# NikolausDemmel/rootba

Hardware: NVIDIA H100
Metric: ms/LM-iter (linearize+QR+PCG) on BAL at 1/2/4/8 H100 vs CPU ref (lower is better)
Workload: dtype f32

## Files before the change

### rootba_b200/csrc/assembled.cuh

```cuda
#pragma once

#include "kernels.cuh"

namespace rba {

template <class S>
__global__ void __launch_bounds__(256) k_rcs_terms(const S* __restrict__ panel, const AsmTerm* __restrict__ terms, long long nt,
                                                   int damping, S* __restrict__ stage, const int* __restrict__ done) {
  using V2 = typename ST<S>::V2;
  if (*done) return;
  const int lane = threadIdx.x & 31;
  const int g = lane / 9, p = lane - 9 * g;
  if (lane >= 27) return;
  const long long warps = (long long)gridDim.x * (blockDim.x >> 5);
  for (long long w = 3 * (blockIdx.x * (long long)(blockDim.x >> 5) + (threadIdx.x >> 5)) + g; w < nt; w += 3 * warps) {
    const AsmTerm at = terms[w];
    const int n = at.meta & 0x7fff, lg = (at.meta >> 15) & 7, KP = at.meta >> 18, G = 1 << lg;
    const int ia = at.ij & 0xffff, ib = at.ij >> 16;
    const int ca = 9 * ia + p, pa = ca >> 1;
    const int off_a = 2 * ((pa >> lg) * 32 + (pa & (G - 1))) + (ca & 1);
    const int cb0 = 9 * ib, pb0 = cb0 >> 1;
    const bool odd = cb0 & 1;
    int off_b[5];
#pragma unroll
    for (int k = 0; k < 5; ++k) off_b[k] = ((pb0 + k) >> lg) * 32 + ((pb0 + k) & (G - 1));
    const size_t rstride = (size_t)KP * 64;
    const S* __restrict__ lmp = panel + at.base;
    const int r0 = damping ? 2 * n - 3 : 0, r1 = damping ? 2 * n : 2 * n - 3;
    S acc[9];
#pragma unroll
    for (int q = 0; q < 9; ++q) acc[q] = 0;
#pragma unroll 3
    for (int r = r0; r < r1; ++r) {
      const S* row = lmp + (size_t)r * rstride;
      const V2* row2 = reinterpret_cast<const V2*>(row);
      const S va = __ldg(row + off_a);
      V2 b[5];
#pragma unroll
      for (int k = 0; k < 5; ++k) b[k] = __ldg(row2 + off_b[k]);
      const S el[10] = {b[0].x, b[0].y, b[1].x, b[1].y, b[2].x, b[2].y, b[3].x, b[3].y, b[4].x, b[4].y};
#pragma unroll
      for (int q = 0; q < 9; ++q) acc[q] = fma(va, odd ? el[q + 1] : el[q], acc[q]);
    }
    S* o = stage + 81 * (size_t)w + 9 * p;
#pragma unroll
    for (int q = 0; q < 9; ++q) o[q] = acc[q];
  }
}

template <class S>
__global__ void k_rcs_combine(const int* __restrict__ blk_ptr, const int* __restrict__ wpos, int nblk, const S* __restrict__ stage,
                              S* __restrict__ out, const int* __restrict__ done) {
  if (*done) return;
  const long long i = blockIdx.x * (long long)blockDim.x + threadIdx.x;
  if (i >= 81LL * nblk) return;
  const int bi = (int)(i / 81), e = (int)(i - 81LL * bi);
  const S* st = stage + e;
  S s = 0;
  for (int t = blk_ptr[bi]; t < blk_ptr[bi + 1]; ++t) s += st[81 * (size_t)wpos[t]];
  out[i] = s;
}

constexpr int DMP_WARPS = 4;
constexpr int DMP_BATCH = 16;
template <class S>
__global__ void __launch_bounds__(DMP_WARPS * 32) k_rcs_damping(const int* __restrict__ blk_ptr, const int2* __restrict__ terms, int nblk,
                                                                 const S* __restrict__ dmp, const S* __restrict__ base,
                                                                 const int2* __restrict__ pos, S* __restrict__ out,
                                                                 const int* __restrict__ done) {
  constexpr int B = DMP_BATCH, NV = 28 * sizeof(S) / 16;
  constexpr int ROUNDS = (2 * B * NV + 31) / 32;
  __shared__ __align__(16) S rec[DMP_WARPS][B][2][28];
  if (*done) return;
  const int w = threadIdx.x >> 5, lane = threadIdx.x & 31;
  const int bi = blockIdx.x * DMP_WARPS + w;
  if (bi >= nblk) return;
  const bool own = lane < 27;
  const int p = lane / 3, q = 3 * (lane - 3 * p);
  S s[3] = {0, 0, 0};
  if (own) {
#pragma unroll
    for (int u = 0; u < 3; ++u) s[u] = base[81 * (size_t)bi + 3 * lane + u];
  }
  int4* rv = reinterpret_cast<int4*>(&rec[w][0][0][0]);
  const int t1 = blk_ptr[bi + 1];
  for (int t0 = blk_ptr[bi]; t0 < t1; t0 += B) {
    const int nb = min(B, t1 - t0);
    int4 v[ROUNDS];
#pragma unroll
    for (int c = 0; c < ROUNDS; ++c) {
      const int i = lane + 32 * c, r = i / NV, k = i - r * NV;
      v[c] = make_int4(0, 0, 0, 0);
      if (i < 2 * nb * NV) {
        const int2 tt = __ldg(terms + t0 + (r >> 1));
        v[c] = __ldg(reinterpret_cast<const int4*>(dmp + 28 * (size_t)(r & 1 ? tt.y : tt.x)) + k);
      }
    }
#pragma unroll
    for (int c = 0; c < ROUNDS; ++c)
      if (lane + 32 * c < 2 * nb * NV) rv[lane + 32 * c] = v[c];
    __syncwarp();
    if (own) {
      for (int j = 0; j < nb; ++j) {
        const S* a = rec[w][j][0];
        const S* b = rec[w][j][1];
#pragma unroll
        for (int u = 0; u < 3; ++u) {
          S t = fma(a[p], b[q + u], S(0));
          t = fma(a[9 + p], b[9 + q + u], t);
          t = fma(a[18 + p], b[18 + q + u], t);
          s[u] += t;
        }
      }
    }
    __syncwarp();
  }
  if (own) {
    S* o = out + 81 * (size_t)pos[bi].x + 3 * lane;
#pragma unroll
    for (int u = 0; u < 3; ++u) o[u] = s[u];
  }
}

template <class S>
__global__ void k_rcs_mirror(const int2* __restrict__ pos, int nblk, S* val, const int* __restrict__ done) {
  if (*done) return;
  const long long i = blockIdx.x * (long long)blockDim.x + threadIdx.x;
  if (i >= 81LL * nblk) return;
  const int bi = (int)(i / 81), e = (int)(i - 81LL * bi);
  const int2 ps = pos[bi];
  if (ps.y >= 0) val[81 * (size_t)ps.y + e] = val[81 * (size_t)ps.x + 9 * (e % 9) + e / 9];
}

constexpr int SPMV_NS = 3;
template <class S>
__global__ void __launch_bounds__(SPMV_CLASSES * 32) k_rcs_spmv(const SpmvChunk* __restrict__ chunks, const int* __restrict__ chunk_ptr,
                                                                 const int* __restrict__ col, const S* __restrict__ val,
                                                                 const S* __restrict__ x, S* __restrict__ y, const int* done, int pdl) {
  constexpr int CH = SPMV_STAGE_BYTES / (81 * (int)sizeof(S)), U = CH / SPMV_CLASSES;
  constexpr int VB = CH * 81 * (int)sizeof(S) + 16;
  constexpr int XWIN = sizeof(S) == 4 ? 256 : 128;
  static_assert(CH % SPMV_CLASSES == 0 && VB % 16 == 0 && XWIN >= CH, "k_rcs_spmv stage layout");
// ... 127 lines not shown
```

### rootba_b200/csrc/layout.hpp

```cpp
#pragma once

#include <algorithm>
#include <cmath>
#include <cstdint>
#include <limits>
#include <numeric>
#include <string>
#include <utility>
#include <vector>

namespace rba {

struct TileInfo {
  long long panel_off;
  int slot_base;
  int lm_base;
  short n;
  short G;
  short KP;
  short nvalid;
};

struct MatvecItem {
  int tile;
// ... 237 lines not shown
    if (!L.csr_y_is_obs) build_csr(nc, L.nyslots, ycam, L.csr_y);
    L.pb_cam_item_ptr.assign(nc + 1, 0);
    for (int c = 0; c < nc; ++c) {
      L.pb_cam_item_ptr[c] = (int)L.pb_items.size();
      for (int b = L.csr_obs.cam_ptr[c]; b < L.csr_obs.cam_ptr[c + 1]; b += PB_SEG_LEN)
        L.pb_items.push_back({c, b, std::min(b + PB_SEG_LEN, L.csr_obs.cam_ptr[c + 1])});
    }
    L.pb_cam_item_ptr[nc] = (int)L.pb_items.size();
  }
  for (const TileInfo& T : L.tiles) {
    const int W = 32 / T.G;
    const int CS = (2 * T.G * T.KP) | 1;
    L.k4_scratch_per_warp = std::max(L.k4_scratch_per_warp, T.KP > kp_max ? 2 * 64 * (int)T.KP : W * CS);
  }
  return "";
}

struct IntPair {
  int x, y;
};

struct PairList {
  std::vector<int> slot0, nn;
  std::vector<IntPair> blk_cam;
  std::vector<int> blk_ptr;
  std::vector<IntPair> terms;
  std::vector<int> wpos;
};

inline std::string build_pair_list(const Layout& L, PairList& P) {
  const int nl = L.nl_local, nc = L.nc;
  P = PairList();
  P.slot0.resize(nl); P.nn.resize(nl);
  long long nt = 0;
  for (int lm = 0; lm < nl; ++lm) {
    const int sidx = L.sorted_of_lm[lm];
    const TileInfo& T = L.tiles[L.tile_of_sorted[sidx]];
    P.slot0[lm] = T.slot_base + (sidx - T.lm_base) * T.n;
    P.nn[lm] = T.n;
    nt += (long long)T.n * (T.n + 1) / 2;
  }
  if (nt > std::numeric_limits<int>::max()) return "more than 2^31 camera-pair terms";
  std::vector<IntPair> raw;
  raw.reserve((size_t)nt);
  for (int lm = 0; lm < nl; ++lm)
    for (int a = 0; a < P.nn[lm]; ++a)
      for (int b = 0; b <= a; ++b) raw.push_back({P.slot0[lm] + a, P.slot0[lm] + b});
  std::vector<int> idx(raw.size()), tmp(raw.size());
  std::iota(idx.begin(), idx.end(), 0);
  std::vector<long long> cnt((size_t)nc + 1);
  auto pass = [&](const std::vector<int>& src, std::vector<int>& dst, bool by_a) {
    std::fill(cnt.begin(), cnt.end(), 0LL);
    for (int w : src) ++cnt[L.slot_cam[by_a ? raw[w].x : raw[w].y] + 1];
    for (int c = 0; c < nc; ++c) cnt[c + 1] += cnt[c];
    for (int w : src) dst[cnt[L.slot_cam[by_a ? raw[w].x : raw[w].y]]++] = w;
  };
  pass(idx, tmp, false);
  pass(tmp, idx, true);
  tmp.clear(); tmp.shrink_to_fit();
  P.terms.resize(raw.size());
  for (size_t t = 0; t < idx.size(); ++t) P.terms[t] = raw[idx[t]];
  P.wpos.swap(idx);
  for (size_t t = 0; t < P.terms.size(); ++t) {
    const IntPair cc{L.slot_cam[P.terms[t].x], L.slot_cam[P.terms[t].y]};
    if (t == 0 || cc.x != P.blk_cam.back().x || cc.y != P.blk_cam.back().y) {
      P.blk_cam.push_back(cc);
      P.blk_ptr.push_back((int)t);
    }
  }
  P.blk_ptr.push_back((int)P.terms.size());
  return "";
}

struct AsmTerm {
  long long base;
  int ij, meta;
};
inline AsmTerm pack_asm_term(long long base, int ia, int ib, int n, int G, int KP) {
  int lg = 0;
  while ((1 << lg) < G) ++lg;
  return {base, ia | ib << 16, n | lg << 15 | KP << 18};
}

constexpr long long ASM_STAGE_BYTES = (long long)2 << 30;

inline int asm_switch_iteration(long long nt, long long panel_scalars, long long s_bytes, int scalar_size) {
  const double staged = 4.0 * (double)nt * 81 * scalar_size, saved = (double)panel_scalars * scalar_size - (double)s_bytes;
  return 1 + (int)std::ceil(2.0 * staged / std::max(saved, 1.0));
}

constexpr int SPMV_CLASSES = 4;
constexpr int SPMV_STAGE_BYTES = 32 * 81 * 4;
constexpr int spmv_chunk_blocks(int scalar_size) { return SPMV_STAGE_BYTES / (81 * scalar_size); }
struct SpmvChunk {
  int row, kb, ke;
  int flags;
};
constexpr int SPMV_FIRST = 1, SPMV_LAST = 2;
struct SpmvDeal {
  int ctas = 0;
  std::vector<int> chunk_ptr;
  std::vector<SpmvChunk> chunks;
};
inline void deal_spmv(const std::vector<int>& row_ptr, int ctas, int chunk_blocks, SpmvDeal& D) {
  D = SpmvDeal();
  const int nrows = (int)row_ptr.size() - 1;
  D.ctas = std::max(1, std::min(ctas, nrows));
  std::vector<long long> cost((size_t)std::max(nrows, 0));
  for (int r = 0; r < nrows; ++r) cost[r] = row_ptr[r + 1] - row_ptr[r];
  const std::vector<int> order = deal_lpt(cost, D.ctas);
  D.chunk_ptr.assign((size_t)D.ctas + 1, 0);
  for (int b = 0; b < D.ctas; ++b) {
    D.chunk_ptr[b] = (int)D.chunks.size();
    for (size_t k = b; k < order.size(); k += D.ctas) {
      const int r = order[k];
      if (r < 0) break;
      const int k0 = row_ptr[r], k1 = row_ptr[r + 1];
      int kb = k0;
      do {
        const int ke = std::min(k1, kb + chunk_blocks);
        D.chunks.push_back({r, kb, ke, (kb == k0 ? SPMV_FIRST : 0) | (ke == k1 ? SPMV_LAST : 0)});
        kb = ke;
      } while (kb < k1);
    }
  }
  D.chunk_ptr[D.ctas] = (int)D.chunks.size();
}

struct AsmPlan {
  long long nt = 0, nblk = 0, nnzb = 0, s_bytes = 0, device_bytes = 0;
  bool fits = false;
  int switch_iteration = 0;
  std::vector<int> row_ptr;
  std::vector<int> col;
  std::vector<IntPair> pos;
  std::vector<AsmTerm> terms;
  SpmvDeal spmv;
};

inline void plan_assembled(const Layout& L, const PairList& P, int scalar_size, AsmPlan& A, int spmv_ctas = 0) {
  A = AsmPlan();
  const int nc = L.nc;
  A.nblk = (long long)P.blk_cam.size();
  A.nt = (long long)P.terms.size();
  long long ndiag = 0;
  for (const IntPair& c : P.blk_cam) ndiag += c.x == c.y;
  A.nnzb = 2 * A.nblk - ndiag;
  A.s_bytes = A.nnzb * 81 * scalar_size;
  A.switch_iteration = asm_switch_iteration(A.nt, L.panel_scalars, A.s_bytes, scalar_size);
  A.fits = 4 * A.s_bytes <= L.panel_scalars * scalar_size && 81 * A.nt * scalar_size <= ASM_STAGE_BYTES;
  if (!A.fits) return;
  A.device_bytes = A.s_bytes + 16 + (A.nblk + A.nt) * 81 * scalar_size + A.nt * (long long)(sizeof(AsmTerm) + sizeof(int) + sizeof(IntPair)) +
                   (A.nblk + 1 + A.nnzb) * (long long)sizeof(int) + A.nblk * (long long)sizeof(IntPair);
  A.row_ptr.assign((size_t)nc + 1, 0);
  A.col.resize((size_t)A.nnzb);
  for (const IntPair& c : P.blk_cam) { ++A.row_ptr[c.x + 1]; if (c.x != c.y) ++A.row_ptr[c.y + 1]; }
  for (int c = 0; c < nc; ++c) A.row_ptr[c + 1] += A.row_ptr[c];
  std::vector<int> fill(A.row_ptr.begin(), A.row_ptr.end() - 1);
  A.pos.resize((size_t)A.nblk);
  for (long long b = 0; b < A.nblk; ++b) {
    const IntPair c = P.blk_cam[b];
    const int lo = fill[c.x]++;
    A.col[lo] = c.y;
    int up = -1;
    if (c.x != c.y) { up = fill[c.y]++; A.col[up] = c.x; }
    A.pos[b] = {lo, up};
  }
  A.terms.reserve((size_t)A.nt);
  for (int lm = 0; lm < L.nl_local; ++lm) {
    const int sidx = L.sorted_of_lm[lm];
    const TileInfo& T = L.tiles[L.tile_of_sorted[sidx]];
    const int g = sidx - T.lm_base;
    for (int a = 0; a < T.n; ++a)
      for (int b = 0; b <= a; ++b) A.terms.push_back(pack_asm_term(T.panel_off + 2LL * g * T.G, a, b, T.n, T.G, T.KP));
  }
  if (spmv_ctas > 0) {
    deal_spmv(A.row_ptr, spmv_ctas, spmv_chunk_blocks(scalar_size), A.spmv);
    A.device_bytes += (long long)A.spmv.chunks.size() * (long long)sizeof(SpmvChunk) + (A.spmv.ctas + 1) * (long long)sizeof(int);
  }
}

}
```

### rootba_b200/csrc/solver.cu

```cuda
#include <cuda_runtime.h>
#include <dlfcn.h>

#include <cstdio>
#include <cstdlib>
#include <cstring>
#include <chrono>
#include <array>
#include <limits>
#include <memory>
#include <string>
#include <utility>
#include <vector>

#include "../../include/rootba_b200.h"
#include "../host/bal_io_fast.hpp"
#include "kernels.cuh"
#include "covariance.cuh"
#include "assembled.cuh"
#include "groups.cuh"
#include "nccl_dyn.hpp"

namespace rba {

thread_local std::string g_err;
// ... 136 lines not shown
    double error[6];
    int error_flags[4];
    int linearize_flags[4];
    double l_diff;
    int apply_flags[4];
  };
  PinnedResults* h_res = nullptr;
  cudaEvent_t poll_ev[2] = {nullptr, nullptr};
  bool linearized = false;
  bool new_linearization_point = false;
  bool have_inc = false;
  S last_lambda = 0;
  bool damping_valid = false;
  struct HeldTerm {
    std::vector<uint8_t> host;
    DeviceBuffer<uint8_t> flags;
    bool all = false;
  } held;
  struct CameraPriorTerm {
    bool on = false;
    DeviceBuffer<S> mean;
    DeviceBuffer<S> L;
    DeviceBuffer<S> A;
    DeviceBuffer<S> r;
    DeviceBuffer<S> H;
    DeviceBuffer<S> g;
    void adopt(CameraPriorTerm& o) { mean.take(o.mean); L.take(o.L); A.take(o.A); r.take(o.r); H.take(o.H); g.take(o.g); }
  } cprior;
  struct PairPriorTerm {
    int n = 0;
    DeviceBuffer<int> ij;
    DeviceBuffer<S> mean;
    DeviceBuffer<S> L;
    DeviceBuffer<S> A;
    DeviceBuffer<S> r;
    DeviceBuffer<int> item;
    DeviceBuffer<int> nbr;
    DeviceBuffer<S> O;
    DeviceBuffer<int> ptr;
    DeviceBuffer<S> ov;
    void adopt(PairPriorTerm& o) { ij.take(o.ij); mean.take(o.mean); L.take(o.L); A.take(o.A); r.take(o.r); item.take(o.item);
                                   nbr.take(o.nbr); O.take(o.O); ptr.take(o.ptr); ov.take(o.ov); }
  } pprior;
  struct LandmarkPriorTerm {
    int n = 0;
    DeviceBuffer<int> slot;
    DeviceBuffer<int> of_lm;
    DeviceBuffer<int> lm;
    DeviceBuffer<S> mean, L, Lg;
    void adopt(LandmarkPriorTerm& o) { slot.take(o.slot); of_lm.take(o.of_lm); lm.take(o.lm); mean.take(o.mean); L.take(o.L); Lg.take(o.Lg); }
  } lprior;
  struct GroupTerm {
    int n = 0;
    std::vector<int> host_lead;
    DeviceBuffer<int> lead, ptr, mem;
    DeviceBuffer<uint8_t> fixed;
    DeviceBuffer<S> ve, y;
    void adopt(GroupTerm& o) { lead.take(o.lead); ptr.take(o.ptr); mem.take(o.mem); fixed.take(o.fixed); ve.take(o.ve); y.take(o.y); }
  } grp;
  struct ObservationTerm {
    bool on = false;
    DeviceBuffer<S> W;
    bool loss_on = false;
    DeviceBuffer<S> loss;
  } obs;
  rba_stage_timings tm{};
  EventPair ev_stage1, ev_stage2, ev_precond, ev_pcg, ev_backsub, ev_update, ev_error, ev_mv, ev_user;
  long long launches = 0;
  long long lin_l0 = 0, solve_l0 = 0, apply_l0 = 0;
  NcclApi* nccl = nullptr;
  ncclComm_t comm = nullptr;
  char* peer_mem = nullptr;
  size_t peer_bytes = 0;
  PeerComm pc{};
  bool peer_ok = false;
  int ar_seq = 0, c_seq = 0, s_seq = 0;
  std::vector<void*> ipc_opened;
  bool cov_ready = false;
  int cov_nblk = 0;
  IntPair* d_cov_blk_cam = nullptr; int* d_cov_blk_ptr = nullptr; IntPair* d_cov_terms = nullptr;
  int* d_cov_lm_slot0 = nullptr; int* d_cov_lm_n = nullptr;
  bool asm_on = false, su_valid = false, s_valid = false, su_new = false;
  int asm_nblk = 0, asm_switch = 0; long long asm_nt = 0, asm_nnzb = 0;
  AsmTerm* d_asm_terms = nullptr; int* d_asm_wpos = nullptr; int* d_asm_blk_ptr = nullptr; IntPair* d_asm_pos = nullptr;
  IntPair* d_asm_slots = nullptr;
  int* d_asm_col = nullptr;
  S* d_asm_stage = nullptr; S* d_asm_Su = nullptr; S* d_asm_S = nullptr;
  SpmvChunk* d_spmv_chunks = nullptr; int* d_spmv_chunk_ptr = nullptr; int spmv_grid = 0, spmv_cap = 0;
  bool s_fresh = false;

  ~Solver() override {
    if (comm && nccl) nccl->CommDestroy(comm);
    for (void* p : ipc_opened) cudaIpcCloseMemHandle(p);
    if (h_prog) cudaFreeHost(h_prog);
    if (h_state) cudaFreeHost(h_state);
    if (h_res) cudaFreeHost(h_res);
    for (EventPair* e : {&ev_stage1, &ev_stage2, &ev_precond, &ev_pcg, &ev_backsub, &ev_update, &ev_error, &ev_mv, &ev_user}) {
      if (e->a) cudaEventDestroy(e->a);
      if (e->b) cudaEventDestroy(e->b);
    }
    for (auto& e : poll_ev) if (e) cudaEventDestroy(e);
    if (stream) cudaStreamDestroy(stream);
  }

  template <class T>
  int alloc(DeviceBuffer<T>& b, size_t count, bool zero, bool counted = true) {
    const size_t bytes = std::max<size_t>(count, 1) * sizeof(T);
    void* q = nullptr;
    CU(cudaMalloc(&q, bytes));
    b = DeviceBuffer<T>((T*)q, count);
    if (counted) device_bytes += bytes;
    if (zero) CU(cudaMemsetAsync(q, 0, bytes, stream));
    return RBA_OK;
  }
  template <class T>
  int copy_in(T* dst, const std::vector<T>& v) {
    if (!v.empty()) CU(cudaMemcpyAsync(dst, v.data(), v.size() * sizeof(T), cudaMemcpyHostToDevice, stream));
    return RBA_OK;
  }
  template <class T>
  int dalloc(T** p, size_t count, bool zero = true, bool counted = true) {
    DeviceBuffer<char> b;
    TRY(alloc(b, std::max<size_t>(count, 1) * sizeof(T), zero, counted));
    *p = (T*)b.get();
    owned.push_back(std::move(b));
    return RBA_OK;
  }
  template <class T>
  int upload(T** p, const std::vector<T>& v, bool counted = true) {
    TRY(dalloc(p, v.size(), false, counted));
    return copy_in(*p, v);
  }
  template <class T>
  int fit(DeviceBuffer<T>& next, const DeviceBuffer<T>& cur, size_t count, const std::vector<T>* src = nullptr) {
    if (!cur.get() || cur.size() < count) TRY(alloc(next, count, false));
    return src ? copy_in(next.get() ? next.get() : cur.get(), *src) : RBA_OK;
  }

  int start(EventPair& e) { e.used = true; CU(cudaEventRecord(e.a, stream)); return RBA_OK; }
  int stop(EventPair& e) { CU(cudaEventRecord(e.b, stream)); return RBA_OK; }
  static double elapsed(EventPair& e) {
    if (!e.used) return 0.0;
    float ms = 0;
    if (cudaEventElapsedTime(&ms, e.a, e.b) != cudaSuccess) return 0.0;
    return 1e-3 * ms;
  }

  int init(const rba_problem_view* pv, const rba_solver_opts* o) {
    TRY(validate_options(*o));
    int ndev = 0;
    if (cudaGetDeviceCount(&ndev) != cudaSuccess || ndev == 0) {
      g_err = "no CUDA device: rootba_b200 has no CPU fallback";
      return RBA_ERR_NO_DEVICE;
    }
    if (opt.device >= 0) CU(cudaSetDevice(opt.device));
    CU(cudaGetDevice(&device));
    cudaDeviceProp prop;
    CU(cudaGetDeviceProperties(&prop, device));
    sm_count = prop.multiProcessorCount;
    CU(cudaStreamCreateWithFlags(&stream, cudaStreamNonBlocking));
    for (EventPair* e : {&ev_stage1, &ev_stage2, &ev_precond, &ev_pcg, &ev_backsub, &ev_update, &ev_error, &ev_mv, &ev_user}) {
      CU(cudaEventCreate(&e->a));
      CU(cudaEventCreate(&e->b));
    }
    for (auto& e : poll_ev) CU(cudaEventCreateWithFlags(&e, cudaEventDisableTiming));
    read_test_hooks();
    TRY(upload_layout(pv));
// ... 1286 lines not shown
    out->num_observations_local = L.nobs_local;
    out->sum_n2 = L.sum_n2;
    out->max_n = L.max_n;
    out->num_tiles = (int)L.tiles.size();
    out->panel_scalars = L.panel_scalars;
    out->panel_scalars_algorithmic = 18 * L.sum_n2;
    out->device_bytes = (int64_t)device_bytes;
    out->matvec_algorithmic_bytes = handover() == Handover::Assembled ? (81 * asm_nnzb + 18 * (int64_t)nc) * (int64_t)sizeof(S) + 4 * (asm_nnzb + nc + 1)
                                                                        : (18 * L.sum_n2 + 18 * L.nobs_local) * (int64_t)sizeof(S) + 4 * L.nobs_local;
    out->landmark_begin = L.lm_begin;
    out->landmark_end = L.lm_end;
    out->num_matvec_items = (int)L.items.size();
    return RBA_OK;
  }

  int get_scaling(void* scaling, void* diag2) override {
    if (scaling) CU(cudaMemcpyAsync(scaling, D.scaling, (size_t)9 * nc * sizeof(S), cudaMemcpyDeviceToHost, stream));
    if (diag2) CU(cudaMemcpyAsync(diag2, D.diag2, (size_t)9 * nc * sizeof(S), cudaMemcpyDeviceToHost, stream));
    CU(cudaStreamSynchronize(stream));
    return RBA_OK;
  }
  int get_rhs(void* b) override {
    CU(cudaMemcpyAsync(b, D.b, (size_t)9 * nc * sizeof(S), cudaMemcpyDeviceToHost, stream));
    CU(cudaStreamSynchronize(stream));
    return RBA_OK;
  }
  int get_precond(void* inv, void* blocks) override {
    if (inv) CU(cudaMemcpyAsync(inv, D.inv, (size_t)81 * nc * sizeof(S), cudaMemcpyDeviceToHost, stream));
    if (blocks) CU(cudaMemcpyAsync(blocks, D.blocks, (size_t)81 * nc * sizeof(S), cudaMemcpyDeviceToHost, stream));
    CU(cudaStreamSynchronize(stream));
    return RBA_OK;
  }
  int right_multiply(const void* x, void* y) override {
    if (!linearized || !damping_valid) { g_err = "rba_right_multiply needs rba_linearize + rba_solve first"; return RBA_ERR_STATE; }
    CU(cudaMemcpyAsync(D.z, x, (size_t)9 * nc * sizeof(S), cudaMemcpyHostToDevice, stream));
    TRY(matvec_launch(D.z, true));
    TRY(allreduce(D.y, (size_t)9 * nc));
    k_pcg_q<S><<<NPART, 128, 0, stream>>>(D, D.y, D.z, D.y, last_lambda);
    ++launches;
    CU(cudaMemcpyAsync(y, D.y, (size_t)9 * nc * sizeof(S), cudaMemcpyDeviceToHost, stream));
    CU(cudaStreamSynchronize(stream));
    CU(cudaGetLastError());
    return RBA_OK;
  }

  int time_matvec(int reps, double* sec) override {
    if (!linearized || !damping_valid) { g_err = "rba_time_matvec needs rba_linearize + rba_solve first"; return RBA_ERR_STATE; }
    TRY(matvec_launch(D.p, false));
    TRY(start(ev_mv));
    for (int r = 0; r < reps; ++r) TRY(matvec_launch(D.p, false));
    TRY(stop(ev_mv));
    CU(cudaStreamSynchronize(stream));
    CU(cudaGetLastError());
    *sec = elapsed(ev_mv) / std::max(reps, 1);
    tm.matvec_time = *sec;
    return RBA_OK;
  }

  int timer_start() override { return start(ev_user); }
  int timer_stop(double* sec) override {
    int rc = stop(ev_user); if (rc) return rc;
    CU(cudaStreamSynchronize(stream));
    *sec = elapsed(ev_user);
    return RBA_OK;
  }
  void* stream_ptr() override { return (void*)stream; }
  int synchronize() override { CU(cudaStreamSynchronize(stream)); return RBA_OK; }

  bool asm_candidate() const { return asm_hook && opt.nranks == 1 && panels; }
  int setup_assembled() {
    if (!asm_candidate()) return RBA_OK;
    PairList P;
    const std::string msg = build_pair_list(L, P);
    if (!msg.empty()) { g_err = msg; return RBA_ERR_UNSUPPORTED; }
    int occ = 0;
    CU(cudaOccupancyMaxActiveBlocksPerMultiprocessor(&occ, k_rcs_spmv<S>, SPMV_CLASSES * 32, 0));
    AsmPlan A;
    const int ctas = std::max(1, occ) * sm_count;
    plan_assembled(L, P, sizeof(S), A, spmv_cap > 0 ? std::min(spmv_cap, ctas) : ctas);
    if (!A.fits) return RBA_OK;
    size_t free_b = 0, total_b = 0;
    CU(cudaMemGetInfo(&free_b, &total_b));
    if ((size_t)A.device_bytes + ((size_t)256 << 20) > free_b) return RBA_OK;
    TRY(upload(&d_asm_terms, A.terms));
    TRY(upload(&d_asm_wpos, P.wpos));
    TRY(upload(&d_asm_slots, P.terms));
    TRY(upload(&d_asm_blk_ptr, P.blk_ptr));
    TRY(upload(&d_asm_pos, A.pos));
    TRY(upload(&d_asm_col, A.col));
    TRY(upload(&d_spmv_chunks, A.spmv.chunks));
    TRY(upload(&d_spmv_chunk_ptr, A.spmv.chunk_ptr));
    spmv_grid = A.spmv.ctas;
    TRY(dalloc(&d_asm_stage, (size_t)A.nt * 81, false));
    TRY(dalloc(&d_asm_Su, (size_t)A.nblk * 81));
    TRY(dalloc(&d_asm_S, (size_t)A.nnzb * 81 + 16 / sizeof(S)));
    asm_nt = A.nt; asm_nblk = (int)A.nblk; asm_nnzb = A.nnzb;
    asm_switch = asm_at > 0 ? asm_at : A.switch_iteration;
    asm_on = true;
    return RBA_OK;
  }
  void assemble(int damping) {
    const int* done = &d_state->done;
    const unsigned per_entry = (unsigned)((81LL * asm_nblk + 255) / 256);
    if (damping) {
      k_rcs_damping<S><<<(asm_nblk + DMP_WARPS - 1) / DMP_WARPS, DMP_WARPS * 32, 0, stream>>>(
          d_asm_blk_ptr, (const int2*)d_asm_slots, asm_nblk, D.dmp, d_asm_Su, (const int2*)d_asm_pos, d_asm_S, done);
      k_rcs_mirror<S><<<per_entry, 256, 0, stream>>>((const int2*)d_asm_pos, asm_nblk, d_asm_S, done);
    } else {
      const int grid = (int)std::max<long long>(1, std::min<long long>((asm_nt + 23) / 24, (long long)sm_count * 16));
      k_rcs_terms<S><<<grid, 256, 0, stream>>>(D.panel, d_asm_terms, asm_nt, 0, d_asm_stage, done);
      k_rcs_combine<S><<<per_entry, 256, 0, stream>>>(d_asm_blk_ptr, d_asm_wpos, asm_nblk, d_asm_stage, d_asm_Su, done);
    }
    launches += 2;
  }

  int cov_build_lists() {
    if (cov_ready) return RBA_OK;
    PairList P;
    const std::string msg = build_pair_list(L, P);
    if (!msg.empty()) { g_err = msg; return RBA_ERR_UNSUPPORTED; }
    TRY(upload(&d_cov_blk_cam, P.blk_cam, false));
    TRY(upload(&d_cov_blk_ptr, P.blk_ptr, false));
    TRY(upload(&d_cov_terms, P.terms, false));
    TRY(upload(&d_cov_lm_slot0, P.slot0, false));
    TRY(upload(&d_cov_lm_n, P.nn, false));
    cov_nblk = (int)P.blk_cam.size();
    cov_ready = true;
    return RBA_OK;
  }
  template <bool TA, bool TB>
  void cov_gemm(long long M, long long N, long long K, double alpha, const double* A, long long lda, const double* B, long long ldb,
                double beta, double* C, long long ldc, int lower, int ktri) {
    k_cov_dgemm<TA, TB><<<dim3((unsigned)(M / COV_TB), (unsigned)(N / COV_TB)), 256, 0, stream>>>((int)M, (int)N, (int)K, alpha, A, lda, B,
                                                                                                   ldb, beta, C, ldc, lower, ktri);
  }
  int cov_copy(double* dst, long long dld, const double* src, long long sld, long long rows, long long cols) {
    CU(cudaMemcpy2DAsync(dst, dld * sizeof(double), src, sld * sizeof(double), rows * sizeof(double), cols, cudaMemcpyDeviceToDevice, stream));
    return RBA_OK;
  }
  int cov_group_passes(double* A, long long ld, long long n, int expand) {
    k_cov_group_symmetrize<<<dim3((unsigned)((n + 31) / 32), (unsigned)((n + 7) / 8)), dim3(32, 8), 0, stream>>>(A, ld, n);
    for (int columns = 0; columns < 2; ++columns)
      k_cov_group_pass<<<(unsigned)((n + 255) / 256), 256, 0, stream>>>(A, ld, n, groups(), columns, expand);
    CU(cudaGetLastError());
    return RBA_OK;
  }
  struct CovInverse {
    DeviceBuffer<char> scratch;
    double* A = nullptr;
    double* d = nullptr;
    double* kb = nullptr; double* wl = nullptr; int* rk = nullptr;
    long long np = 0;
  };
  int cov_factor_inverse(const char* fn, const std::vector<size_t>& extra, CovInverse& c, std::vector<char*>& out) {
    if (opt.nranks > 1) {
      g_err = std::string(fn) + ": sharded handles (nranks > 1) are not supported: the reduced camera matrix would need a cross-rank sum";
      return RBA_ERR_UNSUPPORTED;
    }
    TRY(cov_build_lists());
    constexpr long long TB = COV_TB;
    const long long n = 9LL * nc, np = (n + TB - 1) / TB * TB, ns = L.nslots;
    const int nl = L.nl_local, nt = (int)(np / TB), n_lmp = lprior.n;
    size_t total = 0;
    auto carve = [&](size_t bytes) { const size_t o = total; total += (bytes + 255) & ~size_t(255); return o; };
    const size_t o_A = carve((size_t)(np * np) * 8), o_W = carve((size_t)(np * TB) * 8), o_Y = carve((size_t)(np * TB) * 8),
                 o_T = carve((size_t)(TB * TB) * 8), o_d = carve((size_t)np * 8), o_jp = carve((size_t)ns * 18 * 8),
                 o_kb = carve((size_t)ns * 27 * 8), o_wl = carve((size_t)nl * 9 * 8), o_rk = carve((size_t)nl * 4), o_fail = carve(4);
    std::vector<size_t> o_extra;
    for (size_t b : extra) o_extra.push_back(carve(b));
    size_t free_b = 0, total_b = 0;
    CU(cudaMemGetInfo(&free_b, &total_b));
    if (total > free_b) {
      g_err = std::string(fn) + " needs " + std::to_string(total) + " bytes of device memory (a dense " + std::to_string(n) + " x " +
              std::to_string(n) + " float64 reduced camera matrix plus scratch); " + std::to_string(free_b) + " bytes are free";
      return RBA_ERR_UNSUPPORTED;
    }
    TRY(alloc(c.scratch, total, false, false));
    char* base = c.scratch.get();
    double* A = (double*)(base + o_A); double* W = (double*)(base + o_W); double* Y = (double*)(base + o_Y);
    double* Tt = (double*)(base + o_T); double* d = (double*)(base + o_d); double* jp = (double*)(base + o_jp);
    double* kb = (double*)(base + o_kb); double* wl = (double*)(base + o_wl); int* rk = (int*)(base + o_rk);
    int* fail = (int*)(base + o_fail);
    out.clear();
    for (size_t o : o_extra) out.push_back(base + o);
    const int wgrid = std::max(1, std::min((nl + 3) / 4, sm_count * 16));
    c.A = A; c.d = d; c.kb = kb; c.wl = wl; c.rk = rk; c.np = np;
    CU(cudaMemsetAsync(A, 0, (size_t)(np * np) * 8, stream));
    CU(cudaMemsetAsync(fail, 0x7f, 4, stream));
    auto kcov = n_lmp > 0 ? (D.obs_W ? k_cov_landmark<S, true, true> : k_cov_landmark<S, true>)
                          : (D.obs_W ? k_cov_landmark<S, false, true> : k_cov_landmark<S>);
    if (D.obs_loss) kcov = n_lmp > 0 ? kcov_of<true>(D.obs_W, true) : kcov_of<false>(D.obs_W, true);
    kcov<<<wgrid, 128, 0, stream>>>(D, ko, d_cov_lm_slot0, d_cov_lm_n, nl, jp, kb, wl, rk, n_lmp > 0 ? lprior.of_lm.get() : nullptr);
    k_cov_assemble<<<std::max(1, std::min((cov_nblk + 7) / 8, sm_count * 8)), 256, 0, stream>>>(
// ... 443 lines not shown
```

Before: 5.579.

## Stage panel tiles in shared memory via bulk async copies for term assembly

Rewrites the per-term camera-pair outer-product kernel so each CTA processes a whole panel tile. The tile is streamed into shared memory with bulk global-to-shared copies and mbarriers, and each thread computes a register-blocked 9xRP block of a pair's 81 entries, so panel rows are reused across many term pairs instead of re-read from global per term. Work items are precomputed on the host and sorted by cost, and output writes go through shared memory for coalescing. The combine kernel is also batched, prefetching many stage loads with streaming hints. This adds host planning, more dynamic shared memory, and triangular index math per thread.

Result: faster. 5.368, median of 6 (-3.8%).

```diff
diff --git a/rootba_b200/csrc/assembled.cuh b/rootba_b200/csrc/assembled.cuh
--- a/rootba_b200/csrc/assembled.cuh
+++ b/rootba_b200/csrc/assembled.cuh
@@ -5,59 +5,115 @@
 namespace rba {
 
 template <class S>
-__global__ void __launch_bounds__(256) k_rcs_terms(const S* __restrict__ panel, const AsmTerm* __restrict__ terms, long long nt,
-                                                   int damping, S* __restrict__ stage, const int* __restrict__ done) {
-  using V2 = typename ST<S>::V2;
+__global__ void __launch_bounds__(ASM_TILE_THREADS, sizeof(S) == 4 ? 4 : 3)
+    k_rcs_terms(const AsmTileItem* __restrict__ items, const int* __restrict__ tbase, const S* __restrict__ panel,
+                S* __restrict__ stage, const int* __restrict__ done) {
+  constexpr int RP = sizeof(S) == 4 ? 9 : 3, NP = 9 / RP, NE = 9 * RP;
+  static_assert(ASM_TILE_THREADS * NE * (int)sizeof(S) <= ASM_TILE_BYTES, "k_rcs_terms: the store pass reuses the tile buffer");
+  extern __shared__ __align__(128) unsigned char tile_smem[];
+  __shared__ __align__(8) uint64_t bar;
+  __shared__ long long dst[ASM_TILE_THREADS];
   if (*done) return;
-  const int lane = threadIdx.x & 31;
-  const int g = lane / 9, p = lane - 9 * g;
-  if (lane >= 27) return;
-  const long long warps = (long long)gridDim.x * (blockDim.x >> 5);
-  for (long long w = 3 * (blockIdx.x * (long long)(blockDim.x >> 5) + (threadIdx.x >> 5)) + g; w < nt; w += 3 * warps) {
-    const AsmTerm at = terms[w];
-    const int n = at.meta & 0x7fff, lg = (at.meta >> 15) & 7, KP = at.meta >> 18, G = 1 << lg;
-    const int ia = at.ij & 0xffff, ib = at.ij >> 16;
-    const int ca = 9 * ia + p, pa = ca >> 1;
-    const int off_a = 2 * ((pa >> lg) * 32 + (pa & (G - 1))) + (ca & 1);
-    const int cb0 = 9 * ib, pb0 = cb0 >> 1;
-    const bool odd = cb0 & 1;
-    int off_b[5];
-#pragma unroll
-    for (int k = 0; k < 5; ++k) off_b[k] = ((pb0 + k) >> lg) * 32 + ((pb0 + k) & (G - 1));
-    const size_t rstride = (size_t)KP * 64;
-    const S* __restrict__ lmp = panel + at.base;
-    const int r0 = damping ? 2 * n - 3 : 0, r1 = damping ? 2 * n : 2 * n - 3;
-    S acc[9];
-#pragma unroll
-    for (int q = 0; q < 9; ++q) acc[q] = 0;
-#pragma unroll 3
-    for (int r = r0; r < r1; ++r) {
-      const S* row = lmp + (size_t)r * rstride;
-      const V2* row2 = reinterpret_cast<const V2*>(row);
-      const S va = __ldg(row + off_a);
-      V2 b[5];
-#pragma unroll
-      for (int k = 0; k < 5; ++k) b[k] = __ldg(row2 + off_b[k]);
-      const S el[10] = {b[0].x, b[0].y, b[1].x, b[1].y, b[2].x, b[2].y, b[3].x, b[3].y, b[4].x, b[4].y};
-#pragma unroll
-      for (int q = 0; q < 9; ++q) acc[q] = fma(va, odd ? el[q + 1] : el[q], acc[q]);
-    }
-    S* o = stage + 81 * (size_t)w + 9 * p;
-#pragma unroll
-    for (int q = 0; q < 9; ++q) o[q] = acc[q];
+  const AsmTileItem it = items[blockIdx.x];
+  const int KP = it.kp_lg & 0xffff, lg = it.kp_lg >> 16, G = 1 << lg, nv = it.nvalid;
+  const int rows = 2 * it.n - 3, rowlen = 64 * KP;
+  const int cr = ASM_TILE_BYTES / (rowlen * (int)sizeof(S));
+  S* sp = reinterpret_cast<S*>(tile_smem);
+  const bool act = threadIdx.x < it.nu;
+  uint64_t policy;
+  asm volatile("createpolicy.fractional.L2::evict_normal.b64 %0, 1.0;" : "=l"(policy));
+  const S* tile = panel + it.panel_off;
+  auto request = [&](int r0, int nr) {
+    const uint32_t bytes = (uint32_t)(nr * rowlen * (int)sizeof(S));
+    mbar_expect_tx(&bar, bytes);
+    bulk_g2s(sp, tile + (size_t)r0 * rowlen, bytes, &bar, policy);
+  };
+  if (cr > 0 && threadIdx.x == 0) {
+    mbar_init(&bar, 1);
+    mbar_fence_init();
+    request(0, min(cr, rows));
+  }
+  int g = 0, i = 0, a = 0, b = 0, tt = 0;
+  if (act) {
+    const int u = it.u0 + threadIdx.x, v = u / nv;
+    g = u - v * nv; tt = v / NP; i = v - tt * NP;
+    a = (int)((sqrtf(8.f * tt + 1.f) - 1.f) * 0.5f);
+    while (a * (a + 1) / 2 > tt) --a;
+    while ((a + 1) * (a + 2) / 2 <= tt) ++a;
+    b = tt - a * (a + 1) / 2;
+    dst[threadIdx.x] = 81LL * (tbase[it.lm_base + g] + tt) + NE * i;
+  }
+  auto col = [&](int c) { const int pc = c >> 1; return 2 * (G * g + (pc >> lg) * 32 + (pc & (G - 1))) + (c & 1); };
+  int oa[RP], ob[9];
+#pragma unroll
+  for (int j = 0; j < RP; ++j) oa[j] = col(9 * a + RP * i + j);
+#pragma unroll
+  for (int q = 0; q < 9; ++q) ob[q] = col(9 * b + q);
+  S acc[NE];
+#pragma unroll
+  for (int e = 0; e < NE; ++e) acc[e] = 0;
+  auto row_fma = [&](const S* row) {
+    S va[RP], vb[9];
+#pragma unroll
+    for (int j = 0; j < RP; ++j) va[j] = row[oa[j]];
+#pragma unroll
+    for (int q = 0; q < 9; ++q) vb[q] = row[ob[q]];
+#pragma unroll
+    for (int j = 0; j < RP; ++j)
+#pragma unroll
+      for (int q = 0; q < 9; ++q) acc[9 * j + q] = fma(va[j], vb[q], acc[9 * j + q]);
+  };
+  if (cr == 0) {
+    if (act)
+      for (int r = 0; r < rows; ++r) row_fma(tile + (size_t)r * rowlen);
+  } else {
+    __syncthreads();
+    for (int r0 = 0, k = 0; r0 < rows; r0 += cr, ++k) {
+      const int nr = min(cr, rows - r0);
+      if (k > 0 && threadIdx.x == 0) request(r0, nr);
+      mbar_wait(&bar, k & 1);
+      if (act)
+        for (int r = 0; r < nr; ++r) row_fma(sp + r * rowlen);
+      __syncthreads();
+    }
+  }
+  if (cr == 0) __syncthreads();
+  const int w = threadIdx.x >> 5, lane = threadIdx.x & 31;
+  S* wb = sp + w * 32 * NE;
+#pragma unroll
+  for (int e = 0; e < NE; ++e) wb[NE * lane + e] = acc[e];
+  __syncwarp();
+  const int nact = min(32, it.nu - 32 * w);
+  for (int x = lane; x < nact * NE; x += 32) {
+    const int k = x / NE;
+    stage[dst[32 * w + k] + (x - k * NE)] = wb[x];
   }
 }
 
 template <class S>
 __global__ void k_rcs_combine(const int* __restrict__ blk_ptr, const int* __restrict__ wpos, int nblk, const S* __restrict__ stage,
                               S* __restrict__ out, const int* __restrict__ done) {
+  constexpr int D = sizeof(S) == 4 ? 32 : 16;
   if (*done) return;
   const long long i = blockIdx.x * (long long)blockDim.x + threadIdx.x;
   if (i >= 81LL * nblk) return;
   const int bi = (int)(i / 81), e = (int)(i - 81LL * bi);
+  const int t0 = blk_ptr[bi], m = blk_ptr[bi + 1] - t0;
+  S s = 0;
+  int t = 0;
+  const int* wp = wpos + t0;
   const S* st = stage + e;
-  S s = 0;
-  for (int t = blk_ptr[bi]; t < blk_ptr[bi + 1]; ++t) s += st[81 * (size_t)wpos[t]];
+  for (; t + D <= m; t += D) {
+    int w[D];
+#pragma unroll
+    for (int j = 0; j < D; ++j) w[j] = __ldg(wp + t + j);
+    S v[D];
+#pragma unroll
+    for (int j = 0; j < D; ++j) v[j] = __ldcs(st + 81 * (size_t)w[j]);
+#pragma unroll
+    for (int j = 0; j < D; ++j) s += v[j];
+  }
+  for (; t < m; ++t) s += __ldcs(st + 81 * (size_t)wp[t]);
   out[i] = s;
 }
 
diff --git a/rootba_b200/csrc/layout.hpp b/rootba_b200/csrc/layout.hpp
--- a/rootba_b200/csrc/layout.hpp
+++ b/rootba_b200/csrc/layout.hpp
@@ -343,6 +343,49 @@
   return {base, ia | ib << 16, n | lg << 15 | KP << 18};
 }
 
+constexpr int ASM_TILE_THREADS = 128;
+constexpr int ASM_TILE_BYTES = 48 << 10;
+constexpr int asm_unit_rows(int scalar_size) { return scalar_size == 4 ? 9 : 3; }
+struct AsmTileItem {
+  long long panel_off;
+  int lm_base;
+  int u0, nu;
+  int n;
+  int kp_lg;
+  int nvalid;
+};
+inline void asm_tile_items(const Layout& L, int scalar_size, std::vector<AsmTileItem>& items, std::vector<int>& tbase) {
+  const int NP = 9 / asm_unit_rows(scalar_size);
+  std::vector<long long> lm_t((size_t)L.nl_local);
+  long long t = 0;
+  for (int lm = 0; lm < L.nl_local; ++lm) {
+    lm_t[lm] = t;
+    const long long n = L.tiles[L.tile_of_sorted[L.sorted_of_lm[lm]]].n;
+    t += n * (n + 1) / 2;
+  }
+  tbase.assign(L.sorted_lm.size(), 0);
+  for (size_t s = 0; s < L.sorted_lm.size(); ++s)
+    if (L.sorted_lm[s] >= 0) tbase[s] = (int)lm_t[L.sorted_lm[s]];
+  items.clear();
+  std::vector<long long> cost;
+  for (const TileInfo& T : L.tiles) {
+    int lg = 0;
+    while ((1 << lg) < T.G) ++lg;
+    const long long units = (long long)T.n * (T.n + 1) / 2 * NP * T.nvalid;
+    for (long long u0 = 0; u0 < units; u0 += ASM_TILE_THREADS) {
+      items.push_back({T.panel_off, T.lm_base, (int)u0, (int)std::min<long long>(ASM_TILE_THREADS, units - u0), T.n,
+                       T.KP | lg << 16, T.nvalid});
+      cost.push_back((long long)(2 * T.n - 3) * T.KP);
+    }
+  }
+  std::vector<int> idx(items.size());
+  std::iota(idx.begin(), idx.end(), 0);
+  std::stable_sort(idx.begin(), idx.end(), [&](int a, int b) { return cost[a] > cost[b]; });
+  std::vector<AsmTileItem> sorted(items.size());
+  for (size_t k = 0; k < idx.size(); ++k) sorted[k] = items[idx[k]];
+  items.swap(sorted);
+}
+
 constexpr long long ASM_STAGE_BYTES = (long long)2 << 30;
 
 inline int asm_switch_iteration(long long nt, long long panel_scalars, long long s_bytes, int scalar_size) {
@@ -396,6 +439,8 @@
   std::vector<int> col;
   std::vector<IntPair> pos;
   std::vector<AsmTerm> terms;
+  std::vector<AsmTileItem> items;
+  std::vector<int> tbase;
   SpmvDeal spmv;
 };
 
@@ -411,7 +456,9 @@
   A.switch_iteration = asm_switch_iteration(A.nt, L.panel_scalars, A.s_bytes, scalar_size);
   A.fits = 4 * A.s_bytes <= L.panel_scalars * scalar_size && 81 * A.nt * scalar_size <= ASM_STAGE_BYTES;
   if (!A.fits) return;
-  A.device_bytes = A.s_bytes + 16 + (A.nblk + A.nt) * 81 * scalar_size + A.nt * (long long)(sizeof(AsmTerm) + sizeof(int) + sizeof(IntPair)) +
+  asm_tile_items(L, scalar_size, A.items, A.tbase);
+  A.device_bytes = A.s_bytes + 16 + (A.nblk + A.nt) * 81 * scalar_size + A.nt * (long long)(sizeof(int) + sizeof(IntPair)) +
+                   (long long)A.items.size() * (long long)sizeof(AsmTileItem) + (long long)A.tbase.size() * (long long)sizeof(int) +
                    (A.nblk + 1 + A.nnzb) * (long long)sizeof(int) + A.nblk * (long long)sizeof(IntPair);
   A.row_ptr.assign((size_t)nc + 1, 0);
   A.col.resize((size_t)A.nnzb);
diff --git a/rootba_b200/csrc/solver.cu b/rootba_b200/csrc/solver.cu
--- a/rootba_b200/csrc/solver.cu
+++ b/rootba_b200/csrc/solver.cu
@@ -242,7 +242,8 @@
   int* d_cov_lm_slot0 = nullptr; int* d_cov_lm_n = nullptr;
   bool asm_on = false, su_valid = false, s_valid = false, su_new = false;
   int asm_nblk = 0, asm_switch = 0; long long asm_nt = 0, asm_nnzb = 0;
-  AsmTerm* d_asm_terms = nullptr; int* d_asm_wpos = nullptr; int* d_asm_blk_ptr = nullptr; IntPair* d_asm_pos = nullptr;
+  AsmTileItem* d_asm_items = nullptr; int* d_asm_tbase = nullptr; int* d_asm_wpos = nullptr; int* d_asm_blk_ptr = nullptr;
+  IntPair* d_asm_pos = nullptr; int asm_nitems = 0;
   IntPair* d_asm_slots = nullptr;
   int* d_asm_col = nullptr;
   S* d_asm_stage = nullptr; S* d_asm_Su = nullptr; S* d_asm_S = nullptr;
@@ -1695,7 +1696,8 @@
     size_t free_b = 0, total_b = 0;
     CU(cudaMemGetInfo(&free_b, &total_b));
     if ((size_t)A.device_bytes + ((size_t)256 << 20) > free_b) return RBA_OK;
-    TRY(upload(&d_asm_terms, A.terms));
+    TRY(upload(&d_asm_items, A.items));
+    TRY(upload(&d_asm_tbase, A.tbase));
     TRY(upload(&d_asm_wpos, P.wpos));
     TRY(upload(&d_asm_slots, P.terms));
     TRY(upload(&d_asm_blk_ptr, P.blk_ptr));
@@ -1707,7 +1709,8 @@
     TRY(dalloc(&d_asm_stage, (size_t)A.nt * 81, false));
     TRY(dalloc(&d_asm_Su, (size_t)A.nblk * 81));
     TRY(dalloc(&d_asm_S, (size_t)A.nnzb * 81 + 16 / sizeof(S)));
-    asm_nt = A.nt; asm_nblk = (int)A.nblk; asm_nnzb = A.nnzb;
+    CU(cudaFuncSetAttribute(k_rcs_terms<S>, cudaFuncAttributeMaxDynamicSharedMemorySize, ASM_TILE_BYTES));
+    asm_nt = A.nt; asm_nblk = (int)A.nblk; asm_nnzb = A.nnzb; asm_nitems = (int)A.items.size();
     asm_switch = asm_at > 0 ? asm_at : A.switch_iteration;
     asm_on = true;
     return RBA_OK;
@@ -1720,8 +1723,9 @@
           d_asm_blk_ptr, (const int2*)d_asm_slots, asm_nblk, D.dmp, d_asm_Su, (const int2*)d_asm_pos, d_asm_S, done);
       k_rcs_mirror<S><<<per_entry, 256, 0, stream>>>((const int2*)d_asm_pos, asm_nblk, d_asm_S, done);
     } else {
-      const int grid = (int)std::max<long long>(1, std::min<long long>((asm_nt + 23) / 24, (long long)sm_count * 16));
-      k_rcs_terms<S><<<grid, 256, 0, stream>>>(D.panel, d_asm_terms, asm_nt, 0, d_asm_stage, done);
+      if (asm_nitems > 0)
+        k_rcs_terms<S><<<asm_nitems, ASM_TILE_THREADS, ASM_TILE_BYTES, stream>>>(d_asm_items, d_asm_tbase, D.panel,
+                                                                               d_asm_stage, done);
       k_rcs_combine<S><<<per_entry, 256, 0, stream>>>(d_asm_blk_ptr, d_asm_wpos, asm_nblk, d_asm_stage, d_asm_Su, done);
     }
     launches += 2;
```
